# Patryk27/strolle

Hardware: AMD Instinct MI355X
Metric: Mray/s (primary + shadow + GI rays traced per second, whole job) (higher is better)
Workload: dtype f32

## Files before the change

include/strolle_hip.h:

```cpp
#ifndef STROLLE_HIP_H
#define STROLLE_HIP_H

#include <stddef.h>
#include <stdint.h>

#ifdef __cplusplus
extern "C" {
#endif

typedef struct StEngine StEngine;
typedef uint64_t StHandle;

enum StStatus {
    ST_OK = 0,
    ST_ERR_INVALID_ARGUMENT = 1,
    ST_ERR_NO_DEVICE = 2,
    ST_ERR_UNKNOWN_CAMERA = 3,
    ST_ERR_EMPTY_MESH = 4,
    ST_ERR_HIP = 5,
    ST_ERR_ATLAS_FULL = 6,
    ST_ERR_IO = 7,
    ST_ERR_PARSE = 8,
    ST_ERR_UNSUPPORTED = 9,
    ST_ERR_BVH_TOO_DEEP = 10,
// ... 251 lines not shown
int st_camera_set_output_format(StEngine* e, StHandle camera, int format);

typedef struct StTuning {
    uint32_t struct_size;
    uint32_t overlap;
    uint32_t fuse;
    uint32_t fuse_di_head;
    uint32_t fuse_spatial;
    uint32_t fuse_gi_sampling;
    uint32_t fuse_gi_validation;
    uint32_t fuse_gi_reprojection;
    uint32_t fuse_wavelet;
    uint32_t fuse_compose;
    uint32_t preview_both;
    uint32_t variance_in_reproject;
    uint32_t lean_frame;
    uint32_t skip_scratch_stores;
    uint32_t di_head_on_main;
    uint32_t alias_gi_history;
    uint32_t tile_map;
    uint32_t tile_map_denoise;
    int32_t side_priority;
    uint32_t staging;
    uint32_t double_buffer;
    uint32_t packed_base;
    uint32_t tick_timing;
    uint32_t anyhit_fast;
    uint32_t compact_bvh;
    uint32_t allow_deep_bvh;
    uint32_t device_bake;
    uint32_t wide_bvh;
    uint32_t wide_stack_entries;
    uint32_t primary_packets;
} StTuning;
int st_engine_get_tuning(StEngine* e, StTuning* out);
int st_engine_set_tuning(StEngine* e, const StTuning* tuning);

enum StArithmetic { ST_ARITH_FAST = 0, ST_ARITH_EXACT = 1 };
int st_engine_set_arithmetic(StEngine* e, int arithmetic);
int st_engine_get_arithmetic(StEngine* e, int* out);

enum StBufferId {
    ST_BUF_PRIM_GBUFFER_D0_A = 0, ST_BUF_PRIM_GBUFFER_D0_B = 1, ST_BUF_PRIM_GBUFFER_D1_A = 2, ST_BUF_PRIM_GBUFFER_D1_B = 3,
    ST_BUF_PRIM_SURFACE_MAP_A = 4, ST_BUF_PRIM_SURFACE_MAP_B = 5, ST_BUF_REPROJECTION_MAP = 6, ST_BUF_VELOCITY_MAP = 7,
    ST_BUF_DI_RESERVOIRS_0 = 8, ST_BUF_DI_RESERVOIRS_1 = 9, ST_BUF_DI_RESERVOIRS_2 = 10,
    ST_BUF_DI_DIFF_SAMPLES = 11, ST_BUF_DI_DIFF_PREV_COLORS = 12, ST_BUF_DI_DIFF_CURR_COLORS = 13,
    ST_BUF_DI_DIFF_MOMENTS_A = 14, ST_BUF_DI_DIFF_MOMENTS_B = 15, ST_BUF_DI_DIFF_STASH = 16, ST_BUF_DI_SPEC_SAMPLES = 17,
    ST_BUF_GI_D0 = 18, ST_BUF_GI_D1 = 19, ST_BUF_GI_D2 = 20,
    ST_BUF_GI_RESERVOIRS_0 = 21, ST_BUF_GI_RESERVOIRS_1 = 22, ST_BUF_GI_RESERVOIRS_2 = 23, ST_BUF_GI_RESERVOIRS_3 = 24,
    ST_BUF_GI_DIFF_SAMPLES = 25, ST_BUF_GI_DIFF_PREV_COLORS = 26, ST_BUF_GI_DIFF_CURR_COLORS = 27,
    ST_BUF_GI_DIFF_MOMENTS_A = 28, ST_BUF_GI_DIFF_MOMENTS_B = 29, ST_BUF_GI_DIFF_STASH = 30, ST_BUF_GI_SPEC_SAMPLES = 31,
    ST_BUF_REF_HITS = 32, ST_BUF_REF_RAYS = 33, ST_BUF_REF_COLORS = 34,
    ST_BUF_DBG_USED_MEMORY = 35,
    ST_BUF_COUNT = 36
};
int st_camera_read_buffer(StEngine* e, StHandle camera, int buffer_id, void* out, size_t capacity, size_t* written);
int st_camera_write_buffer(StEngine* e, StHandle camera, int buffer_id, const void* data, size_t bytes);
int st_debug_keep_all_planes(StEngine* e, int keep);
int st_camera_buffer_stale(StEngine* e, StHandle camera, int buffer_id, int* stale);
enum StPassBit {
    ST_PASS_PRIM_VISIBILITY = 1u << 0, ST_PASS_FRAME_REPROJECTION = 1u << 1,
    ST_PASS_DI_SAMPLING = 1u << 2, ST_PASS_DI_TEMPORAL = 1u << 3, ST_PASS_DI_SPATIAL_PICK = 1u << 4, ST_PASS_DI_SPATIAL_TRACE = 1u << 5,
    ST_PASS_DI_SPATIAL_SAMPLE = 1u << 6, ST_PASS_DI_RESOLVING = 1u << 7,
    ST_PASS_GI_REPROJECTION = 1u << 8, ST_PASS_GI_SAMPLING_A = 1u << 9, ST_PASS_GI_SAMPLING_B = 1u << 10, ST_PASS_GI_TEMPORAL = 1u << 11,
    ST_PASS_GI_SPATIAL_PICK = 1u << 12, ST_PASS_GI_SPATIAL_TRACE = 1u << 13, ST_PASS_GI_SPATIAL_SAMPLE = 1u << 14,
    ST_PASS_GI_PREVIEW_0 = 1u << 15, ST_PASS_GI_PREVIEW_1 = 1u << 16, ST_PASS_GI_RESOLVING = 1u << 17,
// ... 60 lines not shown
```

rust/strolle-hip/src/ffi.rs:

```rust
#![allow(non_camel_case_types, dead_code)]
use std::ffi::c_void;
use std::os::raw::c_char;

#[repr(C)]
#[derive(Clone, Copy, Default)]
pub struct StMeshTriangle {
    pub positions: [[f32; 3]; 3],
    pub normals: [[f32; 3]; 3],
    pub uvs: [[f32; 2]; 3],
    pub tangents: [[f32; 4]; 3],
}

#[repr(C)]
#[derive(Clone, Copy, Default)]
pub struct StMaterial {
    pub base_color: [f32; 4],
    pub emissive: [f32; 4],
    pub perceptual_roughness: f32,
    pub metallic: f32,
    pub reflectance: f32,
    pub ior: f32,
    pub base_color_texture: u64,
    pub emissive_texture: u64,
    pub metallic_roughness_texture: u64,
// ... 44 lines not shown
#[repr(C)]
#[derive(Clone, Copy, Default)]
pub struct StTuning {
    pub struct_size: u32,
    pub overlap: u32,
    pub fuse: u32,
    pub fuse_di_head: u32,
    pub fuse_spatial: u32,
    pub fuse_gi_sampling: u32,
    pub fuse_gi_validation: u32,
    pub fuse_gi_reprojection: u32,
    pub fuse_wavelet: u32,
    pub fuse_compose: u32,
    pub preview_both: u32,
    pub variance_in_reproject: u32,
    pub lean_frame: u32,
    pub skip_scratch_stores: u32,
    pub di_head_on_main: u32,
    pub alias_gi_history: u32,
    pub tile_map: u32,
    pub tile_map_denoise: u32,
    pub side_priority: i32,
    pub staging: u32,
    pub double_buffer: u32,
    pub packed_base: u32,
    pub tick_timing: u32,
    pub anyhit_fast: u32,
    pub compact_bvh: u32,
    pub allow_deep_bvh: u32,
    pub device_bake: u32,
    pub wide_bvh: u32,
    pub wide_stack_entries: u32,
    pub primary_packets: u32,
}

#[repr(C)]
#[derive(Clone, Copy, PartialEq, Eq, Debug)]
pub struct StDistGrid {
    pub cols: u32,
    pub rows: u32,
    pub row_edge: [u32; 17],
    pub col_edge: [[u32; 17]; 16],
}

#[repr(C)]
#[derive(Clone, Copy, Default, PartialEq, Eq, Debug)]
pub struct StDistRect {
    pub x0: u32,
    pub y0: u32,
    pub x1: u32,
    pub y1: u32,
}

#[repr(C)]
#[derive(Clone, Copy)]
pub struct StDistUniqueId {
    pub internal: [c_char; 128],
}

pub enum StEngine {}

extern "C" {
    pub fn st_engine_create(device_ordinal: i32, out: *mut *mut StEngine) -> i32;
    pub fn st_engine_destroy(e: *mut StEngine);
    pub fn st_last_error() -> *const c_char;
    pub fn st_build_commit() -> *const c_char;
// ... 172 lines not shown
```

strolle_amd/api.py:

```python
from __future__ import annotations

import ctypes as C
import dataclasses
import enum
import math
import os
import sys
from typing import Optional, Sequence

import numpy as np

_HERE = os.path.dirname(os.path.abspath(__file__))
LIB_PATH = os.environ.get("STROLLE_HIP_LIB") or os.path.join(_HERE, "csrc", "libstrolle_hip.so")
if os.environ.get("STROLLE_HIP_LIB"):
    LIB_PATH = os.environ["STROLLE_HIP_LIB"]


class StMeshTriangle(C.Structure):
    _fields_ = [("positions", C.c_float * 9), ("normals", C.c_float * 9), ("uvs", C.c_float * 6), ("tangents", C.c_float * 12)]


class StSkinVertex(C.Structure):
    _fields_ = [("joints", C.c_uint16 * 4), ("weights", C.c_float * 4)]

# ... 26 lines not shown
class StCamera(C.Structure):
    _fields_ = [("mode", C.c_uint32), ("denoise", C.c_uint32), ("depth", C.c_uint32), ("width", C.c_uint32), ("height", C.c_uint32),
                ("pos_x", C.c_uint32), ("pos_y", C.c_uint32), ("_pad", C.c_uint32), ("transform", C.c_float * 16), ("projection", C.c_float * 16)]


class StDistRect(C.Structure):
    _fields_ = [("x0", C.c_uint32), ("y0", C.c_uint32), ("x1", C.c_uint32), ("y1", C.c_uint32)]

    def as_tuple(self):
        return (self.x0, self.y0, self.x1, self.y1)


class StDistGrid(C.Structure):
    _fields_ = [("cols", C.c_uint32), ("rows", C.c_uint32), ("row_edge", C.c_uint32 * 17), ("col_edge", (C.c_uint32 * 17) * 16)]

    def tiles(self):
        return [dist_grid_tile(self, r) for r in range(self.cols * self.rows)]

    def describe(self):
        return {"cols": self.cols, "rows": self.rows, "row_edges": list(self.row_edge[:self.rows + 1]),
                "col_edges": [list(self.col_edge[k][:self.cols + 1]) for k in range(self.rows)]}


class StDistUniqueId(C.Structure):
    _fields_ = [("internal", C.c_char * 128)]


class StTuning(C.Structure):
    _fields_ = [(n, C.c_uint32) for n in ("struct_size", "overlap", "fuse", "fuse_di_head", "fuse_spatial", "fuse_gi_sampling", "fuse_gi_validation",
                                          "fuse_gi_reprojection", "fuse_wavelet", "fuse_compose", "preview_both", "variance_in_reproject",
                                          "lean_frame", "skip_scratch_stores", "di_head_on_main", "alias_gi_history", "tile_map", "tile_map_denoise")] + \
               [("side_priority", C.c_int32)] + \
               [(n, C.c_uint32) for n in ("staging", "double_buffer", "packed_base", "tick_timing", "anyhit_fast", "compact_bvh",
                                          "allow_deep_bvh", "device_bake", "wide_bvh", "wide_stack_entries", "primary_packets")]


class StKernelProfile(C.Structure):
    _fields_ = [("name", C.c_char * 48), ("launches", C.c_uint32), ("total_ms", C.c_float), ("algorithmic_bytes", C.c_double), ("traversal_bytes", C.c_double)]


class StGltfOptions(C.Structure):
    _fields_ = [("first_handle", C.c_uint64), ("first_image_handle", C.c_uint64), ("override_mask", C.c_uint32), ("reflectance", C.c_float),
                ("perceptual_roughness", C.c_float), ("subdivide", C.c_uint32), ("light_radius", C.c_float), ("_pad", C.c_uint32)]


class StGltfSummary(C.Structure):
    _fields_ = [("meshes", C.c_uint32), ("triangles", C.c_uint32), ("materials", C.c_uint32), ("images", C.c_uint32), ("images_dropped", C.c_uint32),
                ("primitives_skipped", C.c_uint32), ("lights", C.c_uint32), ("lights_skipped", C.c_uint32)]


assert C.sizeof(StMeshTriangle) == 144 and C.sizeof(StMaterial) == 88 and C.sizeof(StLight) == 52 and C.sizeof(StCamera) == 160


class StEnvironmentDesc(C.Structure):
    _fields_ = [("struct_size", C.c_uint32), ("flags", C.c_uint32), ("intensity", C.c_float), ("yaw", C.c_float)]


ENV_KEEP_SUN, ENV_UNIFORM_SAMPLING = 1, 2
ENV_CELL_DTYPE = np.dtype([("q", np.float32), ("alias", np.uint32), ("p", np.float32)])


def environment_desc(intensity: float = 1.0, yaw: float = 0.0, keep_sun: bool = False, uniform: bool = False) -> StEnvironmentDesc:
    return StEnvironmentDesc(C.sizeof(StEnvironmentDesc), (ENV_KEEP_SUN if keep_sun else 0) | (ENV_UNIFORM_SAMPLING if uniform else 0),
                             float(intensity), float(yaw))


class Tonemap(enum.IntEnum):
# ... 1081 lines not shown
```

strolle_amd/csrc/k_denoise.hip:

```cpp
#include "k_common.h"

namespace st {
namespace ST_KNS {


struct f2 { float x, y; };
struct i2v { int x, y; };
ST_D f2 mk2(float x, float y) { f2 r; r.x = x; r.y = y; return r; }
ST_D f2 operator+(f2 a, f2 b) { return mk2(a.x + b.x, a.y + b.y); }
ST_D f2 operator-(f2 a, f2 b) { return mk2(a.x - b.x, a.y - b.y); }
ST_D f2 operator*(f2 a, f2 b) { return mk2(a.x * b.x, a.y * b.y); }
ST_D f2 operator*(f2 a, float b) { return mk2(a.x * b, a.y * b); }
ST_D f2 operator*(float a, f2 b) { return mk2(a * b.x, a * b.y); }
ST_D f2 operator+(f2 a, float b) { return mk2(a.x + b, a.y + b); }
ST_D f2 operator-(f2 a) { return mk2(-a.x, -a.y); }
ST_D f2 splat2(float x) { return mk2(x, x); }
ST_D f2 sqrt2(f2 x) { return mk2(fsqrt(x.x), fsqrt(x.y)); }
ST_D float div_by(float x, float d, float inv_d) {
#if ST_FAST_DEVICE
    return x * inv_d;
#else
    return x / d;
#endif
}
ST_D float4 wavelet_resolve(float r, float g, float b, float v, float w, float ww) {
#if ST_FAST_DEVICE
    const float iw = frcp(w);
    return make_float4(r * iw, g * iw, b * iw, v * (iw * iw));
#else
    return make_float4(r / w, g / w, b / w, v / ww);
#endif
}

ST_D f2 exp_pair(f2 x) {
#if ST_FAST_DEVICE
    return mk2(__builtin_amdgcn_exp2f(x.x * 1.44269504088896341f), __builtin_amdgcn_exp2f(x.y * 1.44269504088896341f));
#else
    return mk2(exp_(x.x), exp_(x.y));
#endif
}

__global__ ST_KERNEL_BOUNDS void k_denoise_reproject(const KArgs a, const float4* prev_colors, const float4* prev_moments,
                                                                      const float4* samples, float4* colors, float4* moments) {
    U2 pos;
    if (!resolve_gid(a, false, &pos) || !owns_pixel(a, pos)) return;
    denoise_reproject_pixel(a, pos, tex_read(samples, a, pos), prev_colors, prev_moments, colors, moments);
}
void launch_denoise_reproject(const KArgs& a, const float4* prev_colors, const float4* prev_moments, const float4* samples, float4* colors,
                              float4* moments, hipStream_t s) {
    ST_LAUNCH(k_denoise_reproject, false, s, a, prev_colors, prev_moments, samples, colors, moments);
}

ST_D void variance_short_history(float4 csn, float4 cdi, float4 cgi, const float4* s_sn, const float4* s_l, int lc, int pitch, float* di_var, float* gi_var) {
    const V3 cn = v3(csn.x, csn.y, csn.z);
    const f2 c_sqrt_luma = mk2(fsqrt(luma(xyz(cdi))), fsqrt(luma(xyz(cgi))));
    const float leeway = csn.w * 0.2f, inv_leeway = frcp(leeway);
    f2 sum_l = splat2(0.0f), sum_ll = splat2(0.0f), sum_1 = splat2(0.0f);
    for (int oy = -2; oy <= 2; oy++) {
#pragma unroll
        for (int ox = -3; ox <= 2; ox++) {
            if (ox == -3 && oy == -2) continue;
            const int lt = lc + oy * pitch + ox;
            const float4 ssn = s_sn[lt];
            if (ssn.w == 0.0f) continue;
            const float4 sl = s_l[lt];
            const f2 l = mk2(sl.x, sl.y);
            const f2 d = c_sqrt_luma - mk2(sl.z, sl.w);
            const float diff = fabsf(ssn.w - csn.w);
            const float depth_weight = diff >= leeway ? 0.0f : 1.0f - div_by(diff, leeway, inv_leeway);
            const float normal_weight = pow64_(fmax_(dot(v3(ssn.x, ssn.y, ssn.z), cn), 0.0f));
            const f2 w = exp_pair(-mk2(fabsf(d.x), fabsf(d.y))) * depth_weight * normal_weight;
            sum_l = sum_l + l * w; sum_ll = sum_ll + (l * l) * w; sum_1 = sum_1 + w;
        }
    }
    { const float m1 = fdiv(sum_l.x, sum_1.x), m2 = fdiv(sum_ll.x, sum_1.x); *di_var = fabsf(m2 - m1 * m1) * 4.0f; }
    { const float m1 = fdiv(sum_l.y, sum_1.y), m2 = fdiv(sum_ll.y, sum_1.y); *gi_var = fabsf(m2 - m1 * m1) * 4.0f; }
}

__global__ ST_KERNEL_BOUNDS void k_denoise_variance(const KArgs a, float4* di_out, float4* gi_out) {
    constexpr int RW = 38, RH = 12, PITCH = 40;
    __shared__ float4 s_sn[PITCH * RH];
    __shared__ float4 s_l[PITCH * RH];
    const TileCoord tc = resolve_tile(a, false);
    const uint32_t wave = threadIdx.x >> 6;
    const U2 pos = pixel_in_tile(tc);
    const bool mine = tc.valid && owns_pixel(a, pos);
    const uint32_t center = pos.y * a.width + pos.x;
    float4 csn = f4z(), cdi = f4z(), cdi_m = f4z(), cgi = f4z(), cgi_m = f4z();
    bool slow;
    if (a.variance_in_reproject) {
        slow = mine && ((a.tile_mask[tile_mask_index(a, pos)] >> (threadIdx.x & 63u)) & 1ull) != 0ull;
        if (!__syncthreads_or(slow ? 1 : 0)) return;
        if (slow) { csn = a.sn[center]; cdi = a.di_diff_curr_colors[center]; cgi = a.gi_diff_curr_colors[center]; }
    } else {
        if (mine) { csn = a.sn[center]; cdi = a.di_diff_curr_colors[center]; cdi_m = a.di_diff_moments[center]; cgi = a.gi_diff_curr_colors[center]; cgi_m = a.gi_diff_moments[center]; }
        slow = mine && csn.w != 0.0f && !(cdi_m.x >= 4.0f);
    }
    if (a.variance_in_reproject || __syncthreads_or(slow ? 1 : 0)) {
        const int32_t bx0 = (int32_t)((tc.x - wave) * 8u) - 3, by0 = (int32_t)(tc.y * 8u) - 2;
        for (int i = (int)threadIdx.x; i < RW * RH; i += kBlockThreads) {
            const int ry = i / RW, rx = i - ry * RW;
            const int32_t gx = bx0 + rx, gy = by0 + ry;
            const int li = ry * PITCH + rx;
            if (gx >= 0 && gy >= 0 && gx < (int32_t)a.width && gy < (int32_t)a.height) {
                const uint32_t at = (uint32_t)gy * a.width + (uint32_t)gx;
                const float4 tdi = a.di_diff_curr_colors[at], tgi = a.gi_diff_curr_colors[at];
                const f2 tl = (mk2(tdi.x, tgi.x) * 0.2126f + mk2(tdi.y, tgi.y) * 0.7152f) + mk2(tdi.z, tgi.z) * 0.0722f;
                const f2 ts = sqrt2(tl);
                s_sn[li] = a.sn[at]; s_l[li] = make_float4(tl.x, tl.y, ts.x, ts.y);
            } else {
                s_sn[li] = f4z();
            }
        }
        __syncthreads();
    }
    if (a.variance_in_reproject && !slow) return;
    if (!mine) return;
    if (csn.w == 0.0f) { di_out[center] = cdi; gi_out[center] = cgi; return; }
    float di_var, gi_var;
    if (!slow) {
        di_var = cdi_m.z - sqr(cdi_m.y);
        gi_var = cgi_m.z - sqr(cgi_m.y);
    } else {
        variance_short_history(csn, cdi, cgi, s_sn, s_l, ((int)(pos.y & 7u) + 2) * PITCH + (int)(wave * 8u + (pos.x & 7u)) + 3, PITCH, &di_var, &gi_var);
    }
    di_var = fmax_(di_var, 0.0f);
    gi_var = fmax_(gi_var, 0.0f);
    if (a.variance_in_reproject) {
        reinterpret_cast<float*>(&di_out[center])[3] = di_var;
        reinterpret_cast<float*>(&gi_out[center])[3] = gi_var;
        return;
    }
    di_out[center] = f4(xyz(cdi), di_var);
    gi_out[center] = f4(xyz(cgi), gi_var);
}

struct WaveletCenter {
    float4 sn; V3 n; f2 sqrt_luma, luma_sigma; float leeway, inv_leeway;
    f2 sum_w, sum_r, sum_g, sum_b, sum_v;
};
ST_D f2 sqrt_luma2(float4 di, float4 gi) { return sqrt2((mk2(di.x, gi.x) * 0.2126f + mk2(di.y, gi.y) * 0.7152f) + mk2(di.z, gi.z) * 0.0722f); }
ST_D WaveletCenter wavelet_begin(float4 csn, float4 cdi, float4 cgi, float strength, f2 c_sqrt_luma) {
    WaveletCenter c;
    c.sn = csn; c.n = v3(csn.x, csn.y, csn.z);
    c.sqrt_luma = c_sqrt_luma;
    c.luma_sigma = mk2(lerpf(2.5f, 0.5f, fsqrt(cdi.w)), lerpf(1.0f, 0.0f, fsqrt(cgi.w)));
    c.leeway = csn.w * (0.33f / strength); c.inv_leeway = frcp(c.leeway);
    c.sum_w = splat2(1.0f); c.sum_r = mk2(cdi.x, cgi.x); c.sum_g = mk2(cdi.y, cgi.y); c.sum_b = mk2(cdi.z, cgi.z); c.sum_v = mk2(cdi.w, cgi.w);
    return c;
}
ST_D bool wavelet_shared(const WaveletCenter& c, float4 ssn, float* depth_weight, float* normal_weight) {
    if (ssn.w == 0.0f) return false;
    const float diff = fabsf(ssn.w - c.sn.w);
    *depth_weight = diff >= c.leeway ? 0.0f : 1.0f - div_by(diff, c.leeway, c.inv_leeway);
    *normal_weight = pow64_(fmax_(dot(v3(ssn.x, ssn.y, ssn.z), c.n), 0.0f));
    return !(*depth_weight == 0.0f || *normal_weight == 0.0f);
}
ST_D void wavelet_tap(WaveletCenter& c, float4 sdi, float4 sgi, f2 t_sqrt_luma, float depth_weight, float normal_weight) {
    const f2 r = mk2(sdi.x, sgi.x), g = mk2(sdi.y, sgi.y), b = mk2(sdi.z, sgi.z), v = mk2(sdi.w, sgi.w);
    const f2 d = c.sqrt_luma - t_sqrt_luma;
    const f2 luma_weight = mk2(fabsf(d.x), fabsf(d.y)) * c.luma_sigma;
    const f2 w = exp_pair(-luma_weight) * depth_weight * normal_weight;
    if (w.x > 0.0f && w.y > 0.0f) {
        c.sum_w = c.sum_w + w; c.sum_r = c.sum_r + w * r; c.sum_g = c.sum_g + w * g; c.sum_b = c.sum_b + w * b; c.sum_v = c.sum_v + (w * w) * v;
    } else {
        if (w.x > 0.0f) { c.sum_w.x += w.x; c.sum_r.x += w.x * r.x; c.sum_g.x += w.x * g.x; c.sum_b.x += w.x * b.x; c.sum_v.x += (w.x * w.x) * v.x; }
        if (w.y > 0.0f) { c.sum_w.y += w.y; c.sum_r.y += w.y * r.y; c.sum_g.y += w.y * g.y; c.sum_b.y += w.y * b.y; c.sum_v.y += (w.y * w.y) * v.y; }
// ... 32 lines not shown
    *bx0 = a.col0 / bw;
    const uint32_t bx1 = (c1 + bw - 1u) / bw;
    *groups_x = bx1 > *bx0 ? bx1 - *bx0 : 0u;
    const uint32_t ty0 = a.row0 >> 3, ty1 = (a.row1 + 7u) >> 3;
    *rows = ((ty1 - ty0) * 8u + kWvH - 1u) / kWvH;
}
template <int BW = kWvW>
ST_D WaveletBlock wavelet_block(const KArgs& a) {
    uint32_t bx0, groups_x, rows;
    wavelet_grid(a, BW, &bx0, &groups_x, &rows);
    const uint32_t ty0 = a.row0 >> 3;
    const uint32_t n_blocks = groups_x * rows, b = blockIdx.x;
    uint32_t lin = b;
    if (a.tile_map == 0u) {
        const uint32_t q = n_blocks >> 3, r = n_blocks & 7u, xcd = b & 7u, k = b >> 3;
        lin = (xcd < r ? xcd * (q + 1u) : r * (q + 1u) + (xcd - r) * q) + k;
    } else if (a.tile_map == 2u) {
        const uint32_t chunk = groups_x * 2u * 8u, full = (n_blocks / chunk) * chunk;
        if (b < full) { const uint32_t c = b / chunk, i = b - c * chunk; lin = c * chunk + (i & 7u) * (groups_x * 2u) + (i >> 3); }
    }
    WaveletBlock w;
    const uint32_t gy = lin / groups_x, gx = lin - gy * groups_x;
    w.x0 = (int32_t)((bx0 + gx) * BW); w.y0 = (int32_t)(ty0 * 8u + gy * kWvH);
    w.valid = gy < rows;
    return w;
}
inline uint32_t wavelet_blocks(const KArgs& a, uint32_t block_w = kWvW) {
    uint32_t bx0, groups_x, rows;
    wavelet_grid(a, block_w, &bx0, &groups_x, &rows);
    return groups_x * rows;
}
ST_D bool wavelet_owns(const KArgs& a, int32_t px, int32_t py) { return px >= 0 && py >= 0 && owns_pixel(a, u2((uint32_t)px, (uint32_t)py)); }

void launch_denoise_variance(const KArgs& a, float4* di_out, float4* gi_out, hipStream_t s) { ST_LAUNCH(k_denoise_variance, false, s, a, di_out, gi_out); }

template <int HALO, int P, int BW = kWvW>
ST_D void wavelet_stage(const KArgs& a, const WaveletBlock& blk, const float4* di_in, const float4* gi_in, float4* s_sn, float4* s_di, float4* s_gi) {
    constexpr int WW = BW + 2 * HALO, WH = kWvH + 2 * HALO;
    for (int i = (int)threadIdx.x; i < WW * WH; i += kWvThreads) {
        const int ry = i / WW, rx = i - ry * WW;
        const int32_t gx = blk.x0 - HALO + rx, gy = blk.y0 - HALO + ry;
        const int li = ry * P + rx;
        if (gx >= 0 && gy >= 0 && gx < (int32_t)a.width && gy < (int32_t)a.height) {
            const uint32_t at = (uint32_t)gy * a.width + (uint32_t)gx;
            const float4 tsn = a.sn[at], tdi = di_in[at], tgi = gi_in[at];
            s_sn[li] = tsn; s_di[li] = tdi; s_gi[li] = tgi;
        } else {
            s_sn[li] = f4z();
        }
    }
}

__global__ __launch_bounds__(kWvThreads) void k_denoise_wavelet_12(const KArgs a, float strength0, float strength1, const float4* di_in, float4* di_mid, float4* di_out,
                                                                   const float4* gi_in, float4* gi_mid, float4* gi_out) {
    constexpr int HALO = 3, WW = kWvW + 2 * HALO, WH = kWvH + 2 * HALO, P = 38;
    constexpr int RW = kWvW + 4, RH = kWvH + 4;
    __shared__ float4 s_sn[P * WH];
    __shared__ float4 s_di[P * WH];
    __shared__ float4 s_gi[P * WH];
    const WaveletBlock blk = wavelet_block(a);
    if (!blk.valid) return;
    wavelet_stage<HALO, P>(a, blk, di_in, gi_in, s_sn, s_di, s_gi);
    __syncthreads();
    float4 r_di[2], r_gi[2]; int r_at[2];
#pragma unroll
    for (int it = 0; it < 2; it++) {
        const int idx = (int)threadIdx.x + it * kWvThreads;
// ... 180 lines not shown
```

strolle_amd/csrc/st_engine.cpp:

```cpp
#include "st_engine.h"

namespace st {

thread_local std::string g_last_error;
thread_local LaunchEvents g_launch_events;

StTuning default_tuning() {
    StTuning t{};
    t.struct_size = sizeof(StTuning);
    t.overlap = t.fuse = t.fuse_di_head = t.fuse_spatial = t.fuse_gi_sampling = t.fuse_gi_validation = t.fuse_gi_reprojection = 1u;
    t.fuse_wavelet = t.fuse_compose = t.preview_both = t.variance_in_reproject = t.lean_frame = 1u;
    t.skip_scratch_stores = t.di_head_on_main = t.alias_gi_history = 1u;
    t.tile_map = 1u; t.tile_map_denoise = 2u; t.side_priority = 0;
    t.staging = t.double_buffer = t.packed_base = 1u; t.tick_timing = 0u;
    t.anyhit_fast = 1u; t.compact_bvh = 1u; t.wide_bvh = 1u; t.primary_packets = 1u;
    t.allow_deep_bvh = 0u; t.device_bake = 1u;
    return t;
}
static void tuning_from_environment(StTuning& t) {
    struct Clear { const char* name; uint32_t StTuning::*field; };
    static const Clear clears[] = {
        {"ST_NO_OVERLAP", &StTuning::overlap}, {"ST_NO_FUSE", &StTuning::fuse}, {"ST_NO_FUSE_DI_HEAD", &StTuning::fuse_di_head},
        {"ST_NO_FUSE_SPATIAL", &StTuning::fuse_spatial}, {"ST_NO_FUSE_GI_SAMPLING", &StTuning::fuse_gi_sampling},
        {"ST_NO_FUSE_GI_VALIDATION", &StTuning::fuse_gi_validation}, {"ST_NO_FUSE_GI_REPROJECTION", &StTuning::fuse_gi_reprojection},
        {"ST_NO_FUSE_WAVELET", &StTuning::fuse_wavelet}, {"ST_NO_FUSE_COMPOSE", &StTuning::fuse_compose}, {"ST_NO_PREVIEW_BOTH", &StTuning::preview_both},
        {"ST_NO_VARIANCE_IN_REPROJECT", &StTuning::variance_in_reproject},
        {"ST_KEEP_ALL_PLANES", &StTuning::lean_frame}, {"ST_KEEP_SCRATCH", &StTuning::skip_scratch_stores}, {"ST_NO_GI_ALIAS", &StTuning::alias_gi_history},
        {"ST_NO_STAGING", &StTuning::staging}, {"ST_NO_DOUBLE_BUFFER", &StTuning::double_buffer}, {"ST_NO_PACKED_BASE", &StTuning::packed_base},
        {"ST_NO_ANYHIT_FAST", &StTuning::anyhit_fast}, {"ST_NO_COMPACT_BVH", &StTuning::compact_bvh}, {"ST_NO_WIDE_BVH", &StTuning::wide_bvh}, {"ST_NO_PRIMARY_PACKETS", &StTuning::primary_packets},
    };
    for (const Clear& c : clears) if (const char* v = getenv(c.name)) { if (atoi(v) != 0) t.*c.field = 0u; else if (t.*c.field == 0u) t.*c.field = 1u; }
    struct Value { const char* name; uint32_t StTuning::*field; };
    static const Value values[] = {
        {"ST_DI_HEAD_ON_MAIN", &StTuning::di_head_on_main}, {"ST_TILE_MAP_DENOISE", &StTuning::tile_map_denoise}, {"ST_TICK_TIMING", &StTuning::tick_timing},
        {"ST_ALLOW_DEEP_BVH", &StTuning::allow_deep_bvh}, {"ST_DEVICE_BAKE", &StTuning::device_bake},
    };
    if (const char* v = getenv("ST_TILE_MAP")) t.tile_map = t.tile_map_denoise = (uint32_t)atoi(v);
    for (const Value& c : values) if (const char* v = getenv(c.name)) t.*c.field = (uint32_t)atoi(v);
    if (const char* v = getenv("ST_SIDE_PRIORITY")) t.side_priority = atoi(v);
}

Engine::Engine() {
    GpuLight sun{};
    sun.d0 = make_float4(0, 0, 0, 25.0f); sun.d1 = make_float4(0, 0, 0, INFINITY); sun.d2 = make_float4(b2f(1u), 0, 0, 0);
    light_buffer.push_back(sun);
    light_slot[-1] = 0;
    blue_noise.assign(256 * 256 * 4, 0);
    reset_profile_totals();
    tuning = default_tuning();
    tuning_from_environment(tuning);
    staging.enabled = tuning.staging != 0u;
    if (const char* x = getenv("ST_BLOOM_TAIL_BYTES")) bloom_tail_wanted = atoi(x);
    if (const char* x = getenv("ST_EXP")) exp_flags = (uint32_t)strtoul(x, nullptr, 0);
    if (const char* ex = getenv("ST_EXACT")) if (atoi(ex) != 0) { arithmetic = ST_ARITH_EXACT; L = launchers_exact(); }
}
int Engine::set_tuning(const StTuning& t) {
    if (t.struct_size != sizeof(StTuning)) return fail(ST_ERR_INVALID_ARGUMENT, "StTuning::struct_size does not match this library");
    if (t.tile_map > 2u || t.tile_map_denoise > 2u) return fail(ST_ERR_INVALID_ARGUMENT, "tile_map is 0, 1 or 2");
    if (t.wide_stack_entries != 0u && (t.wide_stack_entries < 8u || t.wide_stack_entries > 56u)) return fail(ST_ERR_INVALID_ARGUMENT, "wide_stack_entries is 0 (default) or 8 ... 56");
    if (t.wide_stack_entries != tuning.wide_stack_entries) wide_stack_rearmed = 0u;
    tuning = t;
    staging.enabled = tuning.staging != 0u;
// ... 29 lines not shown
```

strolle_amd/csrc/st_render.cpp:

```cpp
#include "st_engine.h"

namespace st {

void Engine::release_camera(CameraState& c) {
    c.slab.release(); c.counters.release(); c.tile_mask.release();
    c.side_stream.reset();
    for (Event* e : {&c.ev_di_head, &c.ev_gi_done, &c.ev_prim_ok, &c.ev_frame_done, &c.ev_setup}) e->reset();
    c.have_prev_frame_events = false;
    c.join_present(); c.present_stream.reset();
    for (auto& p : c.present) p = CameraState::PresentSlot();
}

int Engine::present_copy(CameraState& c, const void* src, void* dst, size_t bytes, hipStream_t stream) {
    if (!has_device) return fail(ST_ERR_NO_DEVICE, "present copy on a host-only engine");
    ST_HIP(hipSetDevice(device));
    if (!c.present_stream) ST_HIP(hipStreamCreateWithFlags(&c.present_stream.h, hipStreamNonBlocking));
    CameraState::PresentSlot* slot = nullptr;
    for (auto& p : c.present) if (p.dst == dst) slot = &p;
    if (!slot) { slot = &c.present[c.present_next & 1u]; c.present_next++; }
    if (slot->pending) ST_HIP(hipEventSynchronize(slot->ev_done.h));
    slot->src = src; slot->dst = dst;
    if (int rc = slot->ev_src.record(stream)) return rc;
    if (int rc = slot->ev_src.wait(c.present_stream)) return rc;
    ST_HIP(hipMemcpyAsync(dst, src, bytes, hipMemcpyDeviceToHost, c.present_stream));
// ... 209 lines not shown
        }
        if (!sky_known || known_sun_altitude != sun_altitude) {
            L.launch_atmosphere_sky(static_cast<const float4*>(d_transmittance.ptr), static_cast<const float4*>(d_scattering.ptr), sun_altitude,
                                  static_cast<float4*>(d_sky.ptr), stream);
            sky_known = true; known_sun_altitude = sun_altitude; luts_generated_now = true;
        }
    }
    if (mode == ST_MODE_BVH_HEATMAP) {
        run(KS_BVH_HEATMAP, ST_PASS_BVH_HEATMAP, [&] { L.launch_bvh_heatmap(a, cur); });
    } else if (mode == ST_MODE_REFERENCE) {
        for (uint32_t d = 0; d <= c.desc.depth; d++) {
            run(KS_REF_TRACING, ST_PASS_REF_TRACING, [&] { L.launch_ref_tracing(a, d, cur); });
            run(KS_REF_SHADING, ST_PASS_REF_SHADING, [&] { L.launch_ref_shading(a, seed(SEED_REF_SHADING + d), d, cur); });
        }
        run(KS_REF_SHADING, ST_PASS_REF_SHADING, [&] { L.launch_ref_shading(a, seed(SEED_REF_SHADING + 255u), 255u, cur); });
    } else {
        const bool needs_di = mode == ST_MODE_IMAGE || mode == ST_MODE_DI_DIFFUSE || mode == ST_MODE_DI_SPECULAR;
        const bool needs_gi = mode == ST_MODE_IMAGE || mode == ST_MODE_GI_DIFFUSE || mode == ST_MODE_GI_SPECULAR;
        const bool denoise = c.desc.denoise != 0u;
        const bool any_objects = !instances.empty();
        const bool tracing = c.frame % 6u < 4u;
        const uint32_t gi_source = (tracing && c.frame % 2u == 1u) ? 1u : 0u;
        const uint32_t pseed = seed(SEED_GI_PREVIEW);
        const bool whole_graph = pass_mask == ~0ull;
        const bool gi_runs = needs_gi && any_objects;
        if (c.gi_aliased && gi_runs && !whole_graph) { const int rc = materialize_gi_history(c); if (rc) return rc; }
        const bool swap_gi_history = tuning.alias_gi_history && arithmetic == ST_ARITH_FAST && gi_runs && whole_graph && gi_source == 0u;
        if (gi_runs && whole_graph) c.gi_aliased = false;
        a.gi_skip_history_copy = swap_gi_history ? 1u : 0u;
        a.tile_mask = c.tile_mask.as<unsigned long long>();
        a.gi_late_mask = a.tile_mask ? a.tile_mask + c.tile_mask_tiles() : nullptr; a.gi_preview_late = 0u;
        const bool gi_preview_both = tuning.preview_both && whole_graph && tuning.fuse && gi_runs && a.gi_late_mask;
        a.variance_in_reproject = (tuning.variance_in_reproject && whole_graph && tuning.fuse && tuning.fuse_wavelet && denoise && needs_di && needs_gi && any_objects && a.tile_mask) ? 1u : 0u;
        const bool even_tiles_x = (((a.width + 7u) / 8u) & 1u) == 0u;
        a.lean = 0u;
        if (tuning.lean_frame && arithmetic == ST_ARITH_FAST && whole_graph && tuning.fuse && denoise && any_objects && mode == ST_MODE_IMAGE) {
            a.lean = kLeanPrim | kLeanSamples;
            if (tuning.fuse_gi_reprojection && tracing && even_tiles_x) a.lean |= kLeanGiRes2;
            if (gi_preview_both) a.lean |= kLeanGiMid;
        }
        c.last_lean = a.lean; c.last_lean_composed = false;
        const bool compose_in_wavelet = tuning.fuse_compose && arithmetic == ST_ARITH_FAST && whole_graph && tuning.fuse && denoise && out != nullptr && mode == ST_MODE_IMAGE && any_objects;
        c.last_lean_composed = compose_in_wavelet && a.lean != 0u;
        a.skip_dead_scratch = (tuning.skip_scratch_stores && whole_graph && tuning.fuse && tuning.fuse_spatial && ((((a.width + 7u) / 8u) & 1u) == 0u) && needs_di && denoise && any_objects) ? 1u : 0u;

        auto do_prim = [&] {
            if (tuning.fuse && any_objects) run(KS_PRIM_VISIBILITY_REPROJECTION, ST_PASS_PRIM_VISIBILITY | ST_PASS_FRAME_REPROJECTION, [&] { L.launch_prim_visibility(a, true, deform_table(), deform_posed(), cur); });
            else run(KS_PRIM_VISIBILITY, ST_PASS_PRIM_VISIBILITY, [&] { L.launch_prim_visibility(a, false, deform_table(), deform_posed(), cur); });
            if (any_objects && !tuning.fuse) run(KS_FRAME_REPROJECTION, ST_PASS_FRAME_REPROJECTION, [&] { L.launch_frame_reprojection(a, cur); });
        };
        auto do_di_head = [&] {
            if (tuning.fuse && tuning.fuse_di_head) run(KS_DI_SAMPLING_TEMPORAL, ST_PASS_DI_SAMPLING | ST_PASS_DI_TEMPORAL, [&] { L.launch_di_sampling_temporal(a, seed(SEED_DI_SAMPLING), seed(SEED_DI_TEMPORAL), cur); });
            else {
                run(KS_DI_SAMPLING, ST_PASS_DI_SAMPLING, [&] { L.launch_di_sampling(a, seed(SEED_DI_SAMPLING), cur); });
                run(KS_DI_TEMPORAL, ST_PASS_DI_TEMPORAL, [&] { L.launch_di_temporal(a, seed(SEED_DI_TEMPORAL), cur); });
            }
        };
        auto do_di_tail = [&] {
            const bool even_tiles = (((a.width + 7u) / 8u) & 1u) == 0u;
            if (tuning.fuse && tuning.fuse_spatial && even_tiles) run(KS_DI_SPATIAL_FUSED, ST_PASS_DI_SPATIAL_PICK | ST_PASS_DI_SPATIAL_TRACE | ST_PASS_DI_SPATIAL_SAMPLE, [&] { L.launch_di_spatial_fused(a, seed(SEED_DI_SPATIAL_PICK), seed(SEED_DI_SPATIAL_SAMPLE), cur); });
            else {
                run(KS_DI_SPATIAL_PICK, ST_PASS_DI_SPATIAL_PICK, [&] { L.launch_di_spatial_pick(a, seed(SEED_DI_SPATIAL_PICK), cur); });
                run(KS_DI_SPATIAL_TRACE, ST_PASS_DI_SPATIAL_TRACE, [&] { L.launch_spatial_trace(a, a.di_diff_samples, a.di_diff_curr_colors, a.di_diff_stash, cur); });
                run(KS_DI_SPATIAL_SAMPLE, ST_PASS_DI_SPATIAL_SAMPLE, [&] { L.launch_di_spatial_sample(a, seed(SEED_DI_SPATIAL_SAMPLE), cur); });
            }
            if (tuning.fuse && denoise) { run(KS_DI_RESOLVING_REPROJECT, ST_PASS_DI_RESOLVING | ST_PASS_DENOISE_REPROJECT_DI, [&] { L.launch_di_resolving(a, true, cur); }); di_reprojected = true; }
// ... 172 lines not shown
```

strolle_amd/csrc/st_types.h:

```cpp
#pragma once
#include "st_math.h"

namespace st {

struct GpuCamera {
    M4 projection_view;
    M4 ndc_to_world;
    float4 origin;
    float4 screen;
};
static_assert(sizeof(GpuCamera) == 160, "Camera uniform is 160 B");

struct GpuMaterial {
    float4 base_color, base_color_texture, emissive, emissive_texture;
    float roughness, metallic, reflectance, ior;
    float4 metallic_roughness_texture, normal_map_texture;
};
static_assert(sizeof(GpuMaterial) == 112, "Material is 112 B");

struct GpuLight { float4 d0, d1, d2, d3, prev_d0, prev_d1, prev_d2; };
static_assert(sizeof(GpuLight) == 112, "Light is 112 B");

struct HostTriangle { float4 d0, d1, d2, d3, d4, d5, d6, d7, d8; };
static_assert(sizeof(HostTriangle) == 144, "Triangle is 144 B");
// ... 31 lines not shown

struct PostArgs {
    const float4* src; void* dst;
    uint32_t width, height, out_width, out_height, format, filter;
    float edge_threshold, edge_threshold_min, subpixel;
};

struct BloomArgs {
    const float4* src; void* dst; const float4* base;
    uint32_t sw, sh, dw, dh, format, additive, firefly, threshold_on;
    float factor, clamp, threshold, knee_lo , knee2 , knee_div ;
    DisplayArgs display;
};

struct BloomTailArgs {
    float4* base; uint32_t bw, bh, n, additive, lds_bytes;
    uint32_t w[8], h[8], off[8];
    float factor[8];
};

struct KArgs {
    GpuCamera cam, prev_cam;
    const float4* bvh; const float4* tri_attr;
    const float4* instance_xforms;
    const GpuMaterial* materials; const GpuLight* lights;
    const GpuLight* lights_lds;
    const uint32_t* material_base_packed;
    const uchar4* atlas; const uchar4* blue_noise;
    const float* byte_luts;
    const float4* transmittance_lut; const float4* sky_lut;
    uint32_t bvh_len, n_lights_buf, light_count, atlas_w, atlas_h;
    uint32_t stack_entries;
    unsigned long long* tile_mask; uint32_t variance_in_reproject;
    unsigned long long* gi_late_mask; uint32_t gi_preview_late;
    uint32_t skip_dead_scratch;
    uint32_t gi_skip_history_copy;
    uint32_t lean;
    const float4* gi_mid_src;
    const float4* bvh_c;
    uint32_t bvh_c_root;
    const float4* bvh_w;
    uint32_t bvh_w_leaf_off;
    uint32_t bvh_w_root;
    uint32_t primary_packets;
    uint32_t bvh_w_link_mask;
    uint32_t bvh_w_links16;
    uint32_t* walk_flags;
    uint32_t exp_flags;
    uint32_t anyhit_contract;
    uint32_t count_bytes;
    uint32_t tri_slots;
    float sun_altitude;
    float sun_dir[3];
    float4 *g0, *g1, *sm;
    const float4 *pg0, *pg1, *psm;
    float4* sn; const float4* psn;
    float4 *reprojection, *velocity;
    float4* di_res[3];
    float4 *di_diff_samples, *di_diff_prev_colors, *di_diff_curr_colors, *di_diff_moments, *di_diff_stash, *di_spec_samples;
    const float4* di_diff_prev_moments;
    float4 *gi_d0, *gi_d1, *gi_d2;
    float4* gi_res[4];
    float4 *gi_diff_samples, *gi_diff_prev_colors, *gi_diff_curr_colors, *gi_diff_moments, *gi_diff_stash, *gi_spec_samples;
    const float4* gi_diff_prev_moments;
    float4 *ref_hits, *ref_rays, *ref_colors;
    uint32_t* dbg_used_memory;
// ... 14 lines not shown
```

Baseline: 9741.

## Add sparse per-wave variance kernel driven by tile mask with sliding LDS window

When variance is computed in the reproject pass, the variance launch now only visits 8x8 tiles flagged in the tile mask. It does this with a per-wave kernel that walks four consecutive tiles and skips empty ones via ballot. Consecutive tiles reuse overlapping halo columns in LDS, stored column-major, instead of restaging them. The change avoids launching the full-grid variance kernel when few pixels need the short-history fallback. In exchange it adds a new code path, wave-level fences, and a strided LDS access pattern.

```diff
diff --git a/include/strolle_hip.h b/include/strolle_hip.h
--- a/include/strolle_hip.h
+++ b/include/strolle_hip.h
@@ -307,6 +307,7 @@
     uint32_t wide_bvh;
     uint32_t wide_stack_entries;
     uint32_t primary_packets;
+    uint32_t variance_sparse;
 } StTuning;
 int st_engine_get_tuning(StEngine* e, StTuning* out);
 int st_engine_set_tuning(StEngine* e, const StTuning* tuning);
diff --git a/rust/strolle-hip/src/ffi.rs b/rust/strolle-hip/src/ffi.rs
--- a/rust/strolle-hip/src/ffi.rs
+++ b/rust/strolle-hip/src/ffi.rs
@@ -100,6 +100,7 @@
     pub wide_bvh: u32,
     pub wide_stack_entries: u32,
     pub primary_packets: u32,
+    pub variance_sparse: u32,
 }
 
 #[repr(C)]
diff --git a/strolle_amd/api.py b/strolle_amd/api.py
--- a/strolle_amd/api.py
+++ b/strolle_amd/api.py
@@ -82,7 +82,8 @@
                                           "lean_frame", "skip_scratch_stores", "di_head_on_main", "alias_gi_history", "tile_map", "tile_map_denoise")] + \
                [("side_priority", C.c_int32)] + \
                [(n, C.c_uint32) for n in ("staging", "double_buffer", "packed_base", "tick_timing", "anyhit_fast", "compact_bvh",
-                                          "allow_deep_bvh", "device_bake", "wide_bvh", "wide_stack_entries", "primary_packets")]
+                                          "allow_deep_bvh", "device_bake", "wide_bvh", "wide_stack_entries", "primary_packets",
+                                          "variance_sparse")]
 
 
 class StKernelProfile(C.Structure):
diff --git a/strolle_amd/csrc/k_denoise.hip b/strolle_amd/csrc/k_denoise.hip
--- a/strolle_amd/csrc/k_denoise.hip
+++ b/strolle_amd/csrc/k_denoise.hip
@@ -51,7 +51,7 @@
     ST_LAUNCH(k_denoise_reproject, false, s, a, prev_colors, prev_moments, samples, colors, moments);
 }
 
-ST_D void variance_short_history(float4 csn, float4 cdi, float4 cgi, const float4* s_sn, const float4* s_l, int lc, int pitch, float* di_var, float* gi_var) {
+ST_D void variance_short_history(float4 csn, float4 cdi, float4 cgi, const float4* s_sn, const float4* s_l, int lc, int pitch, int xs, float* di_var, float* gi_var) {
     const V3 cn = v3(csn.x, csn.y, csn.z);
     const f2 c_sqrt_luma = mk2(fsqrt(luma(xyz(cdi))), fsqrt(luma(xyz(cgi))));
     const float leeway = csn.w * 0.2f, inv_leeway = frcp(leeway);
@@ -60,7 +60,7 @@
 #pragma unroll
         for (int ox = -3; ox <= 2; ox++) {
             if (ox == -3 && oy == -2) continue;
-            const int lt = lc + oy * pitch + ox;
+            const int lt = lc + oy * pitch + ox * xs;
             const float4 ssn = s_sn[lt];
             if (ssn.w == 0.0f) continue;
             const float4 sl = s_l[lt];
@@ -122,7 +122,7 @@
         di_var = cdi_m.z - sqr(cdi_m.y);
         gi_var = cgi_m.z - sqr(cgi_m.y);
     } else {
-        variance_short_history(csn, cdi, cgi, s_sn, s_l, ((int)(pos.y & 7u) + 2) * PITCH + (int)(wave * 8u + (pos.x & 7u)) + 3, PITCH, &di_var, &gi_var);
+        variance_short_history(csn, cdi, cgi, s_sn, s_l, ((int)(pos.y & 7u) + 2) * PITCH + (int)(wave * 8u + (pos.x & 7u)) + 3, PITCH, 1, &di_var, &gi_var);
     }
     di_var = fmax_(di_var, 0.0f);
     gi_var = fmax_(gi_var, 0.0f);
@@ -133,6 +133,79 @@
     }
     di_out[center] = f4(xyz(cdi), di_var);
     gi_out[center] = f4(xyz(cgi), gi_var);
+}
+
+constexpr int kVsTiles = 4, kVsCols = 13, kVsRows = 12, kVsKeep = 5;
+ST_D void wave_lds_fence() { __builtin_amdgcn_fence(__ATOMIC_ACQ_REL, "wavefront"); __builtin_amdgcn_wave_barrier(); }
+ST_D unsigned long long wave_read_word(unsigned long long v, int lane) {
+    const uint32_t lo = (uint32_t)__builtin_amdgcn_readlane((int)(uint32_t)v, lane), hi = (uint32_t)__builtin_amdgcn_readlane((int)(uint32_t)(v >> 32), lane);
+    return ((unsigned long long)hi << 32) | lo;
+}
+template <int C0>
+ST_D void variance_stage_tile(const KArgs& a, uint32_t lane, int32_t x0, int32_t y0, float4* s_sn, float4* s_l) {
+    constexpr int NC = kVsCols - C0;
+    for (int i = (int)lane; i < NC * kVsRows; i += 64) {
+        const int ry = i / NC, rx = C0 + (i - ry * NC);
+        const int32_t gx = x0 + rx, gy = y0 + ry;
+        const int li = rx * kVsRows + ry;
+        if (gx >= 0 && gy >= 0 && gx < (int32_t)a.width && gy < (int32_t)a.height) {
+            const uint32_t at = (uint32_t)gy * a.width + (uint32_t)gx;
+            const float4 tdi = a.di_diff_curr_colors[at], tgi = a.gi_diff_curr_colors[at];
+            const f2 tl = (mk2(tdi.x, tgi.x) * 0.2126f + mk2(tdi.y, tgi.y) * 0.7152f) + mk2(tdi.z, tgi.z) * 0.0722f;
+            const f2 ts = sqrt2(tl);
+            s_sn[li] = a.sn[at]; s_l[li] = make_float4(tl.x, tl.y, ts.x, ts.y);
+        } else {
+            s_sn[li] = f4z();
+        }
+    }
+}
+__global__ __launch_bounds__(kBlockThreads, 8) void k_denoise_variance_sparse(const KArgs a, float4* di_out, float4* gi_out) {
+    __shared__ float4 s_sn_waves[kBlockThreads / 64][kVsCols * kVsRows];
+    __shared__ float4 s_l_waves[kBlockThreads / 64][kVsCols * kVsRows];
+    const uint32_t wave = threadIdx.x >> 6, lane = threadIdx.x & 63u;
+    float4* s_sn = s_sn_waves[wave];
+    float4* s_l = s_l_waves[wave];
+    const TileWindow w = tile_window(a, false);
+    const uint32_t tiles_x = (a.width + 7u) >> 3, tiles_y = (a.height + 7u) >> 3;
+    const uint32_t end = (w.ty1 < tiles_y ? w.ty1 : tiles_y) * tiles_x;
+    const uint32_t first = w.ty0 * tiles_x + (blockIdx.x * (uint32_t)(kBlockThreads / 64) + wave) * (uint32_t)kVsTiles;
+    if (first >= end) return;
+    unsigned long long words = 0ull;
+    if (lane < (uint32_t)kVsTiles && first + lane < end) words = a.tile_mask[first + lane];
+    if (__ballot(words != 0ull) == 0ull) return;
+    bool have_left = false;
+#pragma unroll 1
+    for (int k = 0; k < kVsTiles; k++) {
+        const unsigned long long flags = wave_read_word(words, k);
+        const uint32_t t = first + (uint32_t)k, ty = t / tiles_x, tx = t - ty * tiles_x;
+        const U2 pos = u2(tx * 8u + (lane & 7u), ty * 8u + (lane >> 3));
+        const bool slow = ((flags >> lane) & 1ull) != 0ull && owns_pixel(a, pos);
+        if (__ballot(slow) == 0ull) { have_left = false; continue; }
+        const int32_t x0 = (int32_t)(tx * 8u) - 3, y0 = (int32_t)(ty * 8u) - 2;
+        if (have_left && tx != 0u) {
+            constexpr int kFrom = (kVsCols - kVsKeep) * kVsRows, kCount = kVsKeep * kVsRows;
+            float4 ksn = f4z(), kl = f4z();
+            if (lane < (uint32_t)kCount) { ksn = s_sn[kFrom + lane]; kl = s_l[kFrom + lane]; }
+            wave_lds_fence();
+            if (lane < (uint32_t)kCount) { s_sn[lane] = ksn; s_l[lane] = kl; }
+            variance_stage_tile<kVsKeep>(a, lane, x0, y0, s_sn, s_l);
+        } else {
+            variance_stage_tile<0>(a, lane, x0, y0, s_sn, s_l);
+        }
+        have_left = true;
+        wave_lds_fence();
+        if (slow) {
+            const uint32_t center = pos.y * a.width + pos.x;
+            const float4 csn = a.sn[center], cdi = a.di_diff_curr_colors[center], cgi = a.gi_diff_curr_colors[center];
+            if (csn.w != 0.0f) {
+                float di_var, gi_var;
+                variance_short_history(csn, cdi, cgi, s_sn, s_l, ((int)(lane & 7u) + 3) * kVsRows + (int)(lane >> 3) + 2, 1, kVsRows, &di_var, &gi_var);
+                reinterpret_cast<float*>(&di_out[center])[3] = fmax_(di_var, 0.0f);
+                reinterpret_cast<float*>(&gi_out[center])[3] = fmax_(gi_var, 0.0f);
+            }
+        }
+        wave_lds_fence();
+    }
 }
 
 struct WaveletCenter {
@@ -231,7 +304,15 @@
 }
 ST_D bool wavelet_owns(const KArgs& a, int32_t px, int32_t py) { return px >= 0 && py >= 0 && owns_pixel(a, u2((uint32_t)px, (uint32_t)py)); }
 
-void launch_denoise_variance(const KArgs& a, float4* di_out, float4* gi_out, hipStream_t s) { ST_LAUNCH(k_denoise_variance, false, s, a, di_out, gi_out); }
+void launch_denoise_variance(const KArgs& a, float4* di_out, float4* gi_out, hipStream_t s) {
+    if (a.variance_in_reproject && a.variance_sparse) {
+        const LaunchDims d = launch_dims(a, false);
+        const uint32_t words = ((a.width + 7u) >> 3) * (d.tile_y1 - d.tile_y0), per_block = (uint32_t)(kBlockThreads / 64 * kVsTiles);
+        if (d.blocks) ST_KLAUNCH(k_denoise_variance_sparse, dim3((words + per_block - 1u) / per_block), dim3(kBlockThreads), s, a, di_out, gi_out);
+        return;
+    }
+    ST_LAUNCH(k_denoise_variance, false, s, a, di_out, gi_out);
+}
 
 template <int HALO, int P, int BW = kWvW>
 ST_D void wavelet_stage(const KArgs& a, const WaveletBlock& blk, const float4* di_in, const float4* gi_in, float4* s_sn, float4* s_di, float4* s_gi) {
diff --git a/strolle_amd/csrc/st_engine.cpp b/strolle_amd/csrc/st_engine.cpp
--- a/strolle_amd/csrc/st_engine.cpp
+++ b/strolle_amd/csrc/st_engine.cpp
@@ -15,6 +15,7 @@
     t.staging = t.double_buffer = t.packed_base = 1u; t.tick_timing = 0u;
     t.anyhit_fast = 1u; t.compact_bvh = 1u; t.wide_bvh = 1u; t.primary_packets = 1u;
     t.allow_deep_bvh = 0u; t.device_bake = 1u;
+    t.variance_sparse = 1u;
     return t;
 }
 static void tuning_from_environment(StTuning& t) {
@@ -28,6 +29,7 @@
         {"ST_KEEP_ALL_PLANES", &StTuning::lean_frame}, {"ST_KEEP_SCRATCH", &StTuning::skip_scratch_stores}, {"ST_NO_GI_ALIAS", &StTuning::alias_gi_history},
         {"ST_NO_STAGING", &StTuning::staging}, {"ST_NO_DOUBLE_BUFFER", &StTuning::double_buffer}, {"ST_NO_PACKED_BASE", &StTuning::packed_base},
         {"ST_NO_ANYHIT_FAST", &StTuning::anyhit_fast}, {"ST_NO_COMPACT_BVH", &StTuning::compact_bvh}, {"ST_NO_WIDE_BVH", &StTuning::wide_bvh}, {"ST_NO_PRIMARY_PACKETS", &StTuning::primary_packets},
+        {"ST_VARIANCE_FULL_GRID", &StTuning::variance_sparse},
     };
     for (const Clear& c : clears) if (const char* v = getenv(c.name)) { if (atoi(v) != 0) t.*c.field = 0u; else if (t.*c.field == 0u) t.*c.field = 1u; }
     struct Value { const char* name; uint32_t StTuning::*field; };
diff --git a/strolle_amd/csrc/st_render.cpp b/strolle_amd/csrc/st_render.cpp
--- a/strolle_amd/csrc/st_render.cpp
+++ b/strolle_amd/csrc/st_render.cpp
@@ -265,6 +265,7 @@
         a.gi_late_mask = a.tile_mask ? a.tile_mask + c.tile_mask_tiles() : nullptr; a.gi_preview_late = 0u;
         const bool gi_preview_both = tuning.preview_both && whole_graph && tuning.fuse && gi_runs && a.gi_late_mask;
         a.variance_in_reproject = (tuning.variance_in_reproject && whole_graph && tuning.fuse && tuning.fuse_wavelet && denoise && needs_di && needs_gi && any_objects && a.tile_mask) ? 1u : 0u;
+        a.variance_sparse = tuning.variance_sparse ? 1u : 0u;
         const bool even_tiles_x = (((a.width + 7u) / 8u) & 1u) == 0u;
         a.lean = 0u;
         if (tuning.lean_frame && arithmetic == ST_ARITH_FAST && whole_graph && tuning.fuse && denoise && any_objects && mode == ST_MODE_IMAGE) {
diff --git a/strolle_amd/csrc/st_types.h b/strolle_amd/csrc/st_types.h
--- a/strolle_amd/csrc/st_types.h
+++ b/strolle_amd/csrc/st_types.h
@@ -87,6 +87,7 @@
     uint32_t bvh_len, n_lights_buf, light_count, atlas_w, atlas_h;
     uint32_t stack_entries;
     unsigned long long* tile_mask; uint32_t variance_in_reproject;
+    uint32_t variance_sparse;
     unsigned long long* gi_late_mask; uint32_t gi_preview_late;
     uint32_t skip_dead_scratch;
     uint32_t gi_skip_history_copy;
```

Result: no change. 9715 (-0.3%).
